# taipingeric/yolo-v4-tf.keras

Measured on AMD Instinct MI355X. Metric: images/sec end-to-end predict() at 608x608 batch 32; conv MFMA %peak, higher is better.
Workload: dtype bf16

## Files before the change

### yolo-v4-tf.keras_amd/csrc/csp_stage.hip

```cpp
#include "conv_chain.h"

#include "phase_trace.h"

namespace y4 {

#ifdef CS_TRACE
__device__ unsigned long long cs_trace_buf[4 * 8 * 16];
#define CS_TR_WG 8
#define CS_TR_T0 3
#endif

#define CS_SEG(K) do { __builtin_amdgcn_sched_barrier(0); __builtin_amdgcn_s_setprio(K); __builtin_amdgcn_sched_barrier(0); } while (0)

constexpr int CS_W3 = 0;
constexpr int CS_W4 = CS_W3 + 8 * 1024;
constexpr int CS_W2 = CS_W4 + 4 * 1024;
constexpr int CS_W5 = CS_W2 + 8 * 1024;
constexpr int CS_W6 = CS_W5 + 36 * 1024;
constexpr int CS_W7 = CS_W6 + 8 * 1024;
constexpr int CS_WBYTES = CS_W7 + 16 * 1024;
constexpr int CS_A3 = 0, CS_A4 = 128, CS_A2 = 192, CS_A5 = 320, CS_A6 = 448, CS_A7 = 576, CS_AFLOATS = 704;
constexpr int CS_AFF = CS_WBYTES;
constexpr int CS_X1 = CS_AFF + 3 * 1024;
constexpr int CS_HROWS = 336;
constexpr int CS_X4 = CS_X1 + CS_HROWS * 128;
constexpr int CS_LDS = CS_X4 + CS_HROWS * 64;
constexpr int CS_BLOB_BYTES = CS_WBYTES + 3 * 1024;
static_assert(CS_LDS <= 160 * 1024, "LDS budget");
constexpr int CS_WAVES = 8, CS_T = 16, CS_H = CS_T + 2;

struct CspStageK {
    const char* in;
    char* out;
    const char* blob;
    int in_cstride, in_coff, out_cstride, out_coff;
    unsigned in_bytes;
    int N, H, W;
    int tiles_x, tiles_y, tiles_per_img, ntiles;
};

template <int NC>
__device__ __forceinline__ void cs_affine(const float* tab, int cout, int fg, float* sc, float* sh) {
#pragma unroll
    for (int c = 0; c < NC; ++c) {
        const int ch = chunk_channel(0, c, fg);
#pragma unroll
        for (int h = 0; h < 8; h += 4) {
            const f32x4 s4 = *(const f32x4*)(tab + ch + h);
            const f32x4 h4 = *(const f32x4*)(tab + cout + ch + h);
#pragma unroll
            for (int e = 0; e < 4; ++e) { sc[c * 8 + h + e] = s4[e]; sh[c * 8 + h + e] = h4[e]; }
        }
    }
}

template <int NREP>
__device__ __forceinline__ void cs_wfrag(const char* w, int s, int lane, u32x4 (&wf)[NREP]) {
#pragma unroll
    for (int j = 0; j < NREP; ++j) wf[j] = *(const u32x4*)(w + ((s * NREP + j) * 64 + lane) * 16);
}

template <int DT, int NREP>
__device__ __forceinline__ void cs_act_pack(const f32x4 (&acc)[NREP], const float* sc, const float* sh, u32x4* out) {
    float v[NREP * 4];
#pragma unroll
    for (int j = 0; j < NREP; ++j)
        bn_act4<true, Y4_ACT_MISH>(acc[j], sc + j * 4, sh + j * 4, v + j * 4);
#pragma unroll
    for (int c = 0; c < NREP / 2; ++c) Elem<DT>::store_chunk(&out[c], v + c * 8);
}

template <int DT>
__global__ __launch_bounds__(64 * CS_WAVES, 1) void csp_stage_kernel(const CspStageK p) {
    using E = Elem<DT>;
    using T = typename E::type;
    extern __shared__ __attribute__((aligned(16))) char smem[];
    const int tid = threadIdx.x, lane = tid & 63, wave = __builtin_amdgcn_readfirstlane(tid >> 6);
    const int q = lane & 15, g = lane >> 4;
    const float* const aff = (const float*)(smem + CS_AFF);
    char* const X1 = smem + CS_X1;
    char* const X4 = smem + CS_X4;

    const int G = gridDim.x, xcd = blockIdx.x & 7, bi = blockIdx.x >> 3;
    const int nb_x = (G - xcd + 7) >> 3;
    const int t_lo = (int)((int64_t)p.ntiles * xcd / 8), t_hi = (int)((int64_t)p.ntiles * (xcd + 1) / 8);
    int t = t_lo + bi;

    {
        const __amdgpu_buffer_rsrc_t rb = make_rsrc(p.blob, CS_BLOB_BYTES);
        for (int u = wave; u < CS_BLOB_BYTES / 1024; u += CS_WAVES)
            buffer_load16_lds(rb, smem + __builtin_amdgcn_readfirstlane(u * 1024), u * 1024 + lane * 16, 0);
    }
    const __amdgpu_buffer_rsrc_t rs_in = make_rsrc(p.in, p.in_bytes);
    constexpr int CS_NPIECE = (CS_HROWS / 8 + CS_WAVES - 1) / CS_WAVES;
    int lx_rel[CS_NPIECE];
#pragma unroll
    for (int k = 0; k < CS_NPIECE; ++k) {
        const int hp = (wave + CS_WAVES * k) * 8 + (lane >> 3);
        const int hy = hp / CS_H, hx = hp - hy * CS_H;
        const int flags = hp >= CS_H * CS_H ? 15 : ((hy == 0) | ((hy == CS_H - 1) << 1) | ((hx == 0) << 2) | ((hx == CS_H - 1) << 3));
        lx_rel[k] = (((hy * p.W + hx) * p.in_cstride + (((lane & 7) ^ (hp & 7)) * 8)) * 2) | flags;
    }
    auto load_x = [&](int tile) {
        const int n = tile / p.tiles_per_img, rem = tile - n * p.tiles_per_img;
        const int ty = rem / p.tiles_x, tx = rem - ty * p.tiles_x;
        const int base = (((n * p.H + ty * CS_T - 1) * p.W + tx * CS_T - 1) * p.in_cstride + p.in_coff) * 2;
        const int tmask = (ty == 0) | ((ty == p.tiles_y - 1) << 1) | ((tx == 0) << 2) | ((tx == p.tiles_x - 1) << 3);
#pragma unroll
        for (int k = 0; k < CS_NPIECE; ++k) {
            const int u = wave + CS_WAVES * k;
            if (u >= CS_HROWS / 8) break;
            const int off = (lx_rel[k] & tmask) || (lx_rel[k] & 15) == 15 ? (int)0x80000000 : base + (lx_rel[k] & ~15);
            buffer_load16_lds(rs_in, X1 + __builtin_amdgcn_readfirstlane(u * 1024), off, 0);
        }
    };
    if (t < t_hi) load_x(t);

    int xr_main[2];
#pragma unroll
    for (int i = 0; i < 2; ++i) xr_main[i] = (2 * wave + i + 1) * CS_H + 1 + q;
    auto ring_geom = [&](int e, int& hy, int& hx) {
        if (e < 2) { hy = e == 0 ? 0 : CS_H - 1; hx = 1 + q; }
        else {
            const int pp = min((e - 2) * 16 + q, 2 * CS_H - 1);
            hy = pp >> 1; hx = (pp & 1) * (CS_H - 1);
        }
    };
    const int n_extra = wave == 0 ? 2 : wave < 4 ? 1 : 0;

    bool first_tile = true;
#ifdef CS_TRACE
    int tr_i = 0;
    unsigned long long tr_t[16] = {0, 0, 0, 0, 0, 0, 0, 0, 0, 0, 0, 0, 0, 0, 0, 0};
#endif
    for (; t < t_hi; t += nb_x) {
        const int n = t / p.tiles_per_img, rem = t - n * p.tiles_per_img;
        const int ty = rem / p.tiles_x, tx = rem - ty * p.tiles_x;
#ifdef CS_TRACE
        const bool tr_on = blockIdx.x == CS_TR_WG && tr_i >= CS_TR_T0 && tr_i < CS_TR_T0 + 4;
#endif
        PHASE_POINT(0);
        if (first_tile) wait_vmcnt_then_barrier<0>();
        else wait_vmcnt_then_barrier<0>();
        first_tile = false;
        PHASE_POINT(1);
        CS_SEG(3);

        u32x4 C2[2][2], R3[2][2];
        {
            float sc3[16], sh3[16], sc4[8], sh4[8];
            cs_affine<2>(aff + CS_A3, 64, g, sc3, sh3);
            cs_affine<1>(aff + CS_A4, 32, g, sc4, sh4);
            f32x4 a3[2][4], a2[2][4];
#pragma unroll
            for (int i = 0; i < 2; ++i)
#pragma unroll
                for (int j = 0; j < 4; ++j) a3[i][j] = a2[i][j] = f32x4{0.f, 0.f, 0.f, 0.f};
#pragma unroll
            for (int s = 0; s < 2; ++s) {
                u32x4 xf[2], w3[4], w2[4];
#pragma unroll
                for (int i = 0; i < 2; ++i) xf[i] = *(const u32x4*)(X1 + xr_main[i] * 128 + (((s * 4 + g) ^ (xr_main[i] & 7)) * 16));
                cs_wfrag<4>(smem + CS_W3, s, lane, w3);
                cs_wfrag<4>(smem + CS_W2, s, lane, w2);
#pragma unroll
                for (int i = 0; i < 2; ++i)
#pragma unroll
                    for (int j = 0; j < 4; ++j) {
                        Mma<DT>::run(a3[i][j], w3[j], xf[i]);
                        Mma<DT>::run(a2[i][j], w2[j], xf[i]);
                    }
            }
            PHASE_POINT(2);
#pragma unroll
            for (int i = 0; i < 2; ++i) cs_act_pack<DT, 4>(a3[i], sc3, sh3, R3[i]);
            {
                float sc2[16], sh2[16];
                cs_affine<2>(aff + CS_A2, 64, g, sc2, sh2);
#pragma unroll
                for (int i = 0; i < 2; ++i) cs_act_pack<DT, 4>(a2[i], sc2, sh2, C2[i]);
            }
            PHASE_POINT(3);
            CS_SEG(2);
            auto conv4_to_t4 = [&](const u32x4* x3, int xr, int hy, int hx) {
                f32x4 a4[2];
                a4[0] = a4[1] = f32x4{0.f, 0.f, 0.f, 0.f};
#pragma unroll
                for (int s = 0; s < 2; ++s) {
                    u32x4 w4[2];
                    cs_wfrag<2>(smem + CS_W4, s, lane, w4);
#pragma unroll
                    for (int j = 0; j < 2; ++j) Mma<DT>::run(a4[j], w4[j], x3[s]);
                }
                u32x4 pk;
                cs_act_pack<DT, 2>(a4, sc4, sh4, &pk);
                const int gy = ty * CS_T - 1 + hy, gx = tx * CS_T - 1 + hx;
                if (!((unsigned)gy < (unsigned)p.H && (unsigned)gx < (unsigned)p.W)) pk = u32x4{0u, 0u, 0u, 0u};
                *(u32x4*)(X4 + xr * 64 + ((g ^ ((xr >> 1) & 3)) * 16)) = pk;
            };
            for (int ex = 0; ex < n_extra; ++ex) {
                int ex_hy, ex_hx;
                ring_geom(ex == 1 ? 4 : wave, ex_hy, ex_hx);
                const int xr_extra = ex_hy * CS_H + ex_hx;
                u32x4 X3e[2];
                f32x4 a3e[4];
#pragma unroll
                for (int j = 0; j < 4; ++j) a3e[j] = f32x4{0.f, 0.f, 0.f, 0.f};
#pragma unroll
                for (int s = 0; s < 2; ++s) {
                    u32x4 w3[4];
                    const u32x4 xf = *(const u32x4*)(X1 + xr_extra * 128 + (((s * 4 + g) ^ (xr_extra & 7)) * 16));
                    cs_wfrag<4>(smem + CS_W3, s, lane, w3);
#pragma unroll
                    for (int j = 0; j < 4; ++j) Mma<DT>::run(a3e[j], w3[j], xf);
                }
                cs_act_pack<DT, 4>(a3e, sc3, sh3, X3e);
                conv4_to_t4(X3e, xr_extra, ex_hy, ex_hx);
            }
            PHASE_POINT(4);
            CS_SEG(1);
#pragma unroll
            for (int i = 0; i < 2; ++i) conv4_to_t4(R3[i], xr_main[i], 2 * wave + i + 1, 1 + q);
        }
        PHASE_POINT(5);
        asm volatile("s_waitcnt lgkmcnt(0)\n\ts_barrier" ::: "memory");
        PHASE_POINT(6);
        CS_SEG(3);
        if (t + nb_x < t_hi) load_x(t + nb_x);
        PHASE_POINT(7);

        {
            f32x4 a5[2][4];
#pragma unroll
            for (int i = 0; i < 2; ++i)
#pragma unroll
                for (int j = 0; j < 4; ++j) a5[i][j] = f32x4{0.f, 0.f, 0.f, 0.f};
#pragma unroll
            for (int tap = 0; tap < 9; ++tap) {
                const int ky = tap / 3, kx = tap - ky * 3;
                u32x4 xf[2], w5[4];
#pragma unroll
                for (int i = 0; i < 2; ++i) {
                    const int r = (2 * wave + i + ky) * CS_H + q + kx;
                    xf[i] = *(const u32x4*)(X4 + r * 64 + ((g ^ ((r >> 1) & 3)) * 16));
                }
                cs_wfrag<4>(smem + CS_W5, tap, lane, w5);
#pragma unroll
                for (int i = 0; i < 2; ++i)
#pragma unroll
                    for (int j = 0; j < 4; ++j) Mma<DT>::run(a5[i][j], w5[j], xf[i]);
            }
            PHASE_POINT(8);
            u32x4 X5[2][2];
            {
                float sc5[16], sh5[16];
                cs_affine<2>(aff + CS_A5, 64, g, sc5, sh5);
#pragma unroll
                for (int i = 0; i < 2; ++i) {
                    float v[16];
#pragma unroll
                    for (int j = 0; j < 4; ++j)
                        bn_act4<true, Y4_ACT_MISH>(a5[i][j], sc5 + j * 4, sh5 + j * 4, v + j * 4);
#pragma unroll
                    for (int c = 0; c < 2; ++c) {
                        float rv[8];
                        E::load_chunk(&R3[i][c], rv);
#pragma unroll
                        for (int e = 0; e < 8; ++e) v[c * 8 + e] += rv[e];
                    }
#pragma unroll
                    for (int c = 0; c < 2; ++c) E::store_chunk(&X5[i][c], v + c * 8);
                }
            }
            PHASE_POINT(9);
            CS_SEG(2);
            u32x4 Y6[2][2];
            {
                f32x4 a6[2][4];
#pragma unroll
                for (int i = 0; i < 2; ++i)
#pragma unroll
                    for (int j = 0; j < 4; ++j) a6[i][j] = f32x4{0.f, 0.f, 0.f, 0.f};
#pragma unroll
                for (int s = 0; s < 2; ++s) {
                    u32x4 w6[4];
                    cs_wfrag<4>(smem + CS_W6, s, lane, w6);
#pragma unroll
                    for (int i = 0; i < 2; ++i)
#pragma unroll
                        for (int j = 0; j < 4; ++j) Mma<DT>::run(a6[i][j], w6[j], X5[i][s]);
                }
                float sc6[16], sh6[16];
                cs_affine<2>(aff + CS_A6, 64, g, sc6, sh6);
#pragma unroll
                for (int i = 0; i < 2; ++i) cs_act_pack<DT, 4>(a6[i], sc6, sh6, Y6[i]);
            }
            PHASE_POINT(10);
            CS_SEG(1);
            {
                f32x4 a7[2][4];
#pragma unroll
                for (int i = 0; i < 2; ++i)
#pragma unroll
                    for (int j = 0; j < 4; ++j) a7[i][j] = f32x4{0.f, 0.f, 0.f, 0.f};
#pragma unroll
                for (int s = 0; s < 4; ++s) {
                    u32x4 w7[4];
                    cs_wfrag<4>(smem + CS_W7, s, lane, w7);
#pragma unroll
                    for (int i = 0; i < 2; ++i)
#pragma unroll
                        for (int j = 0; j < 4; ++j) Mma<DT>::run(a7[i][j], w7[j], s < 2 ? Y6[i][s] : C2[i][s - 2]);
                }
                PHASE_POINT(11);
                float sc7[16], sh7[16];
                cs_affine<2>(aff + CS_A7, 64, g, sc7, sh7);
#pragma unroll
                for (int i = 0; i < 2; ++i) {
                    u32x4 Z[2];
                    cs_act_pack<DT, 4>(a7[i], sc7, sh7, Z);
                    const int64_t pix = ((int64_t)n * p.H + ty * CS_T + 2 * wave + i) * p.W + tx * CS_T + q;
                    T* op = (T*)p.out + pix * p.out_cstride + p.out_coff;
#pragma unroll
                    for (int c = 0; c < 2; ++c) *(u32x4*)(op + chunk_channel(0, c, g)) = Z[c];
                }
            }
        }
        PHASE_POINT(12);
#ifdef CS_TRACE
        if (tr_on && lane == 0) {
#pragma unroll
            for (int k = 0; k < 13; ++k) cs_trace_buf[((tr_i - CS_TR_T0) * 8 + wave) * 16 + k] = tr_t[k];
        }
        ++tr_i;
#endif
    }
}

PHASE_TRACE_READER(y4_cs_trace_read, cs_trace_buf)

bool csp_stage_supported(int dtype, int h, int w) {
    return dtype != Y4_F32 && h % CS_T == 0 && w % CS_T == 0 && h >= CS_T && w >= CS_T;
}
size_t csp_stage_blob_bytes() { return CS_BLOB_BYTES; }

int csp_stage_launch(int dtype, const void* in, int n, int h, int w, int in_cstride, int in_coff, const void* blob, void* out,
                     int out_cstride, int out_coff, hipStream_t stream) {
    Y4_REQUIRE(csp_stage_supported(dtype, h, w), Y4_EINVAL, "csp_stage: dtype %d / %d x %d map not supported", dtype, h, w);
    Y4_REQUIRE(in && blob && out && n > 0, Y4_EINVAL, "csp_stage: null pointer / empty batch");
    Y4_REQUIRE(in_cstride % 8 == 0 && in_coff % 8 == 0 && out_cstride % 8 == 0 && out_coff % 8 == 0, Y4_EINVAL,
               "csp_stage: views not 16-byte aligned");
    const int64_t in_bytes = (int64_t)n * h * w * in_cstride * 2;
    Y4_REQUIRE(in_bytes < (1ll << 31), Y4_EINVAL, "csp_stage: input (%lld B) exceeds the 2 GiB buffer-descriptor range", (long long)in_bytes);
    CspStageK k{};
    k.in = (const char*)in; k.out = (char*)out; k.blob = (const char*)blob;
    k.in_cstride = in_cstride; k.in_coff = in_coff; k.out_cstride = out_cstride; k.out_coff = out_coff;
    k.in_bytes = (unsigned)in_bytes;
    k.N = n; k.H = h; k.W = w;
    k.tiles_x = w / CS_T; k.tiles_y = h / CS_T; k.tiles_per_img = k.tiles_x * k.tiles_y; k.ntiles = n * k.tiles_per_img;
    int cus = 0;
    if (int r = cu_count(&cus)) return r;
    int grid = cus & ~7;
    if (grid < 8) grid = 8;
    if (grid > ((k.ntiles + 7) & ~7)) grid = (k.ntiles + 7) & ~7;
    return dtype == Y4_BF16 ? launch_lds<csp_stage_kernel<Y4_BF16>>(CS_LDS, dim3(grid), dim3(64 * CS_WAVES), CS_LDS, stream, k)
                            : launch_lds<csp_stage_kernel<Y4_F16>>(CS_LDS, dim3(grid), dim3(64 * CS_WAVES), CS_LDS, stream, k);
}

int pack_csp_stage(int dtype, const float* const* w, const float* const* scale, const float* const* shift, void* blob,
                   hipStream_t stream) {
    Y4_REQUIRE(dtype == Y4_BF16 || dtype == Y4_F16, Y4_EINVAL, "pack_csp_stage: 16-bit dtypes only (got %d)", dtype);
    struct Item { int conv, cout, cin, ksize, woff, aoff; };
    static const Item items[6] = {{2, 64, 64, 1, CS_W2, CS_A2},  {3, 64, 64, 1, CS_W3, CS_A3}, {4, 32, 64, 1, CS_W4, CS_A4},
                                  {5, 64, 32, 3, CS_W5, CS_A5},  {6, 64, 64, 1, CS_W6, CS_A6}, {7, 64, 128, 1, CS_W7, CS_A7}};
    for (int k = 0; k < 6; ++k) {
        const Item& it = items[k];
        Y4_REQUIRE(w[k] && scale[k] && shift[k], Y4_EINVAL, "pack_csp_stage: null pointer for conv %d", it.conv);
        if (int r = pack_frag16(dtype, it.cout, it.cin, it.ksize, w[k], (char*)blob + it.woff, stream)) return r;
        if (int r = copy_affine(it.cout, {scale[k], shift[k]}, (float*)((char*)blob + CS_AFF) + it.aoff, stream)) return r;
    }
    return Y4_OK;
}

}
```

### yolo-v4-tf.keras_amd/csrc/phase_trace.h

```cpp
#pragma once

#if defined(RB_TRACE) || defined(CS_TRACE) || defined(SD_TRACE)
#define PHASE_POINT(P)                                                                                      \
    do {                                                                                                    \
        __builtin_amdgcn_sched_barrier(0);                                                                  \
        if (tr_on) asm volatile("s_memtime %0" : "=s"(tr_t[P]));                                            \
        __builtin_amdgcn_sched_barrier(0);                                                                  \
    } while (0)
#define PHASE_TRACE_READER(NAME, BUF) \
    extern "C" int NAME(unsigned long long* dst) { return (int)hipMemcpyFromSymbol(dst, HIP_SYMBOL(BUF), sizeof(BUF)); }
#else
#define PHASE_POINT(P)
#define PHASE_TRACE_READER(NAME, BUF)
#endif
```

### yolo-v4-tf.keras_amd/csrc/resblock.hip

```cpp
#include <type_traits>

#include "conv_chain.h"

#include "phase_trace.h"

namespace y4 {

#ifdef RB_TRACE
__device__ unsigned long long rb_trace_buf[3 * 8 * 16];
#define RB_TR_WG 8
#define RB_TR_T0 1
#endif

constexpr int RB_T = 16, RB_H = RB_T + 2, RB_WAVES = 8;

template <int C, int TY = RB_T> struct RbGeom {
    static constexpr int HR = TY + 2;
    static constexpr int HROWS = HR * RB_H;
    static constexpr int NFA = HR + (2 * HR + 15) / 16;
    static constexpr int CPR = C / 8;
    static constexpr int ROWB = C * 2 + 16;
    static constexpr int XT_PIECES = (HROWS * (CPR + 1) + 63) / 64;
    static constexpr int NF = C / 16;
    static constexpr int KS1 = C / 32;
    static constexpr int STEP_BYTES = 2 * NF * 1024;
    static constexpr int P = KS1 / 2;
    static constexpr int NSTEPS = 10 * P;
    static constexpr int RING = 4;
    static constexpr int PPW = STEP_BYTES / 1024 / RB_WAVES;
    static constexpr int AFF_BYTES = 4 * C * 4;
    static constexpr int AFF_PAD = (AFF_BYTES + 1023) / 1024 * 1024;
    static constexpr int BLOB_BYTES = AFF_PAD + NSTEPS * STEP_BYTES;
    static constexpr int L_AFF = 0, L_RING = AFF_PAD, L_XT = L_RING + RING * STEP_BYTES;
    static constexpr int XT_SLACK = XT_PIECES * 1024 - HROWS * (CPR + 1) * 16;
    static constexpr int LDS = L_XT + XT_PIECES * 1024 + (XT_SLACK >= TOUCH_LDS ? 0 : 1024);
    static constexpr int L_TOUCH = LDS - TOUCH_LDS;
    static constexpr int WN = NF / 4, WM = RB_WAVES / WN, MREP = TY / WM;
    static_assert(C != 64 || 2 * LDS <= 160 * 1024, "C = 64: two workgroups per compute unit (resblock_dispatch)");
    static_assert(LDS <= 160 * 1024 && MREP >= 1 && MREP * WM == TY && PPW >= 1 && PPW * RB_WAVES * 1024 == STEP_BYTES && NFA <= 3 * RB_WAVES,
                  "resblock geometry");
};

struct ResBlockK {
    const char* in;
    char* out;
    const char* blob;
    int in_cstride, in_coff, out_cstride, out_coff;
    unsigned in_bytes, out_bytes;
    int N, H, W;
    int tiles_x, tiles_y, tiles_per_img, ntiles;
    int t_begin, t_end;
    int touch;
};

template <int DT, int C, int TY>
__global__ __launch_bounds__(64 * RB_WAVES, C == 64 ? 4 : 2) void resblock_kernel(const ResBlockK p) {
    using E = Elem<DT>;
    using G = RbGeom<C, TY>;
    constexpr int PARTS = RB_T / TY;
    constexpr int ROWB = G::ROWB, CPR = G::CPR, NF = G::NF, MREP = G::MREP;
    extern __shared__ __attribute__((aligned(16))) char smem[];
    const int tid = threadIdx.x, lane = tid & 63, wave = __builtin_amdgcn_readfirstlane(tid >> 6);
    const int q = lane & 15, g = lane >> 4;
    const int wm = wave / G::WN, wn = wave - wm * G::WN;
    const float* const aff = (const float*)(smem + G::L_AFF);
    char* const XT = smem + G::L_XT;
    char* const ring = smem + G::L_RING;

    const int GR = gridDim.x, xcd = blockIdx.x & 7, bi = blockIdx.x >> 3;
    const int nb_x = (GR - xcd + 7) >> 3;
    const int span = p.t_end - p.t_begin;
    const int t_lo = p.t_begin + (int)((int64_t)span * xcd / 8), t_hi = p.t_begin + (int)((int64_t)span * (xcd + 1) / 8);
    int t = t_lo + bi;
    auto locate = [&](int u, int& n, int& y_out0, int& tx) {
        const int full = u / PARTS, part = u - full * PARTS;
        n = full / p.tiles_per_img;
        const int rem = full - n * p.tiles_per_img, ty = rem / p.tiles_x;
        tx = rem - ty * p.tiles_x;
        y_out0 = ty * RB_T + part * TY;
    };

    const __amdgpu_buffer_rsrc_t rb = make_rsrc(p.blob, G::BLOB_BYTES);
    const __amdgpu_buffer_rsrc_t rs_in = make_rsrc(p.in, p.in_bytes), rs_out = make_rsrc(p.out, p.out_bytes);
    if (p.touch != 0) weight_touch(rb, smem + G::L_TOUCH, 0, G::BLOB_BYTES, wave, RB_WAVES, lane);
    for (int u = wave; u < G::AFF_PAD / 1024; u += RB_WAVES)
        buffer_load16_lds(rb, smem + __builtin_amdgcn_readfirstlane(u * 1024), u * 1024 + lane * 16, 0);
    auto stage_w = [&](int st) {
        char* const dst = ring + (st & (G::RING - 1)) * G::STEP_BYTES;
#pragma unroll
        for (int k = 0; k < G::PPW; ++k) {
            const int u = wave + k * RB_WAVES;
            buffer_load16_lds(rb, dst + __builtin_amdgcn_readfirstlane(u * 1024), G::AFF_PAD + u * 1024 + lane * 16, st * G::STEP_BYTES);
        }
    };
    auto load_x = [&](int tile) {
        int n, yo, tx;
        locate(tile, n, yo, tx);
        const int y0 = yo - 1, x0 = tx * RB_T - 1;
        constexpr int SPR = CPR + 1, DSLOT = RB_WAVES * 64, DHP = DSLOT / SPR, DCH = DSLOT % SPR, DHY = DHP / RB_H, DHX = DHP % RB_H;
        static_assert(DCH + SPR - 1 < 2 * SPR && DHX + RB_H < 2 * RB_H, "one carry per step");
        int slot0 = wave * 64 + lane;
        asm volatile("" : "+v"(slot0));
        const int hp0 = slot0 / SPR;
        int ch = slot0 - hp0 * SPR, hy = hp0 / RB_H;
        int hx = hp0 - hy * RB_H;
        const int pix_b = p.in_cstride * 2, row_b = p.W * pix_b;
        int off = (((n * p.H + y0) * p.W + x0) * p.in_cstride + p.in_coff) * 2 + hy * row_b + hx * pix_b + ch * 16;
        const int d_off = DHY * row_b + DHX * pix_b + DCH * 16, c_ch = pix_b - SPR * 16, c_hx = row_b - RB_H * pix_b;
#pragma unroll
        for (int k = 0; k * RB_WAVES < G::XT_PIECES; ++k) {
            const int u = wave + k * RB_WAVES;
            if (u < G::XT_PIECES) {
                const bool ok = ch < CPR && hy < G::HR && (unsigned)(y0 + hy) < (unsigned)p.H && (unsigned)(x0 + hx) < (unsigned)p.W;
                buffer_load16_lds(rs_in, XT + __builtin_amdgcn_readfirstlane(u * 1024), ok ? off : (int)0x80000000, 0);
            }
            ch += DCH; hx += DHX; hy += DHY; off += d_off;
            if (ch >= SPR) { ch -= SPR; hx += 1; off += c_ch; }
            if (hx >= RB_H) { hx -= RB_H; hy += 1; off += c_hx; }
        }
    };
    if (t < t_hi) { load_x(t); stage_w(0); stage_w(1); stage_w(2); stage_w(3); }

#ifdef RB_TRACE
    int tr_i = 0;
    unsigned long long tr_t[16] = {0, 0, 0, 0, 0, 0, 0, 0, 0, 0, 0, 0, 0, 0, 0, 0};
#endif
    for (; t < t_hi; t += nb_x) {
        int n, y_out0, tx;
        locate(t, n, y_out0, tx);
#ifdef RB_TRACE
        const bool tr_on = TY == RB_T && C == RB_TRACE && blockIdx.x == RB_TR_WG && tr_i >= RB_TR_T0 && tr_i < RB_TR_T0 + 3;
#endif
        PHASE_POINT(0);
        wait_vmcnt_then_barrier<0>();
        PHASE_POINT(1);

        u32x4 res[MREP][2];

        auto phase_a = [&](auto nfr_c) {
            constexpr int NFR = decltype(nfr_c)::value;
            char* row[NFR];
            bool inside[NFR];
#pragma unroll
            for (int k = 0; k < NFR; ++k) {
                const int f = wave + k * RB_WAVES;
                int hy, hx;
                if (f < G::HR) { hy = f; hx = 1 + q; }
                else { const int pp = min((f - G::HR) * 16 + q, 2 * G::HR - 1); hy = pp >> 1; hx = (pp & 1) * (RB_H - 1); }
                const int r = hy * RB_H + hx;
                row[k] = XT + r * ROWB;
                const int gy = y_out0 - 1 + hy, gx = tx * RB_T - 1 + hx;
                inside[k] = (unsigned)gy < (unsigned)p.H && (unsigned)gx < (unsigned)p.W;
            }
            f32x4 acc[NFR][NF];
#pragma unroll
            for (int k = 0; k < NFR; ++k)
#pragma unroll
                for (int j = 0; j < NF; ++j) acc[k][j] = f32x4{0.f, 0.f, 0.f, 0.f};
#pragma unroll
            for (int s = 0; s < G::KS1; ++s) {
                u32x4 xf[NFR], wf[NF];
#pragma unroll
                for (int k = 0; k < NFR; ++k) xf[k] = *(const u32x4*)(row[k] + (s * 4 + g) * 16);
#pragma unroll
                for (int j = 0; j < NF; ++j) wf[j] = *(const u32x4*)(ring + (s >> 1) * G::STEP_BYTES + (((s & 1) * NF + j) * 64 + lane) * 16);
#pragma unroll
                for (int k = 0; k < NFR; ++k)
#pragma unroll
                    for (int j = 0; j < NF; ++j) Mma<DT>::run(acc[k][j], wf[j], xf[k]);
            }
#pragma unroll
            for (int c = 0; c < NF / 2; ++c) {
                float sc[8], sh[8];
#pragma unroll
                for (int h = 0; h < 8; h += 4) {
                    const int ch = chunk_channel(0, c, g) + h;
                    const f32x4 s4 = *(const f32x4*)(aff + ch), h4 = *(const f32x4*)(aff + C + ch);
#pragma unroll
                    for (int e = 0; e < 4; ++e) { sc[h + e] = s4[e]; sh[h + e] = h4[e]; }
                }
#pragma unroll
                for (int k = 0; k < NFR; ++k) {
                    float v[8];
                    bn_act4<true, Y4_ACT_MISH>(acc[k][2 * c], sc, sh, v);
                    bn_act4<true, Y4_ACT_MISH>(acc[k][2 * c + 1], sc + 4, sh + 4, v + 4);
                    u32x4 pk;
                    E::store_chunk(&pk, v);
                    if (!inside[k]) pk = u32x4{0u, 0u, 0u, 0u};
                    *(u32x4*)(row[k] + (4 * c + g) * 16) = pk;
                }
            }
        };
        if (wave + 2 * RB_WAVES < G::NFA) phase_a(std::integral_constant<int, 3>{});
        else if (wave + RB_WAVES < G::NFA) phase_a(std::integral_constant<int, 2>{});
        else if (wave < G::NFA) phase_a(std::integral_constant<int, 1>{});
        PHASE_POINT(2);
        asm volatile("s_waitcnt lgkmcnt(0)\n\ts_barrier" ::: "memory");
        PHASE_POINT(3);

        {
            int pix[MREP];
#pragma unroll
            for (int i = 0; i < MREP; ++i) {
                const int gy = y_out0 + wm * MREP + i, gx = tx * RB_T + q;
                pix[i] = gy < p.H && gx < p.W ? (n * p.H + gy) * p.W + gx : -1;
            }
            auto load_res = [&]() {
#pragma unroll
                for (int i = 0; i < MREP; ++i) {
                    const int o = pix[i] < 0 ? (int)0x80000000 : (pix[i] * p.in_cstride + p.in_coff) * 2;
#pragma unroll
                    for (int c = 0; c < 2; ++c) res[i][c] = buffer_load16(rs_in, o + chunk_channel(wn * 64, c, g) * 2);
                }
            };
            constexpr int S0 = G::NSTEPS - 4, RES_LOADS = 2 * MREP;
            f32x4 acc[MREP][4];
#pragma unroll
            for (int i = 0; i < MREP; ++i)
#pragma unroll
                for (int j = 0; j < 4; ++j) acc[i][j] = f32x4{0.f, 0.f, 0.f, 0.f};
#pragma unroll
            for (int st = 4; st <= G::P + 3; ++st) stage_w(st);
            const char* const xbase = XT + ((wm * MREP) * RB_H + q) * ROWB + g * 16;
            u32x4 xf[2][MREP], wf[2][4];
            auto read_frags = [&](int buf, int st, int kk) {
                const int ks = st - G::P;
                const int cb = ks / 9, tap = ks - cb * 9;
                const int ky = tap / 3, kx = tap - ky * 3;
                const char* const wst = ring + (st & (G::RING - 1)) * G::STEP_BYTES;
#pragma unroll
                for (int i = 0; i < MREP; ++i) {
                    xf[buf][i] = *(const u32x4*)(xbase + ((i + ky) * RB_H + kx) * ROWB + (cb * 8 + kk * 4) * 16);
                }
#pragma unroll
                for (int j = 0; j < 4; ++j) wf[buf][j] = *(const u32x4*)(wst + ((kk * NF + wn * 4 + j) * 64 + lane) * 16);
            };
            auto mma = [&](int buf) {
#pragma unroll
                for (int i = 0; i < MREP; ++i)
#pragma unroll
                    for (int j = 0; j < 4; ++j)
                        Mma<DT>::run(acc[i][j], wf[buf][j], xf[buf][i]);
            };
            PHASE_POINT(4);
            read_frags(0, G::P, 0);
#pragma unroll
            for (int st = G::P; st < G::NSTEPS; ++st) {
                if (st == G::P + 3 * G::P) PHASE_POINT(5);
                if (st == G::P + 6 * G::P) PHASE_POINT(6);
                if (st == S0) load_res();
                read_frags(1, st, 1);
                __builtin_amdgcn_sched_barrier(0);
                mma(0);
                __builtin_amdgcn_sched_barrier(0);
                if (st + 1 < G::NSTEPS) {
                    constexpr int LAST = G::NSTEPS - 1;
                    const int younger = (st + 3 < LAST ? st + 3 : LAST) - (st + 1);
                    const int extra = st >= S0 && st <= S0 + 2 ? RES_LOADS : 0;
                    static_assert(S0 > G::P && 2 * G::PPW + RES_LOADS < 64, "window of the residual's loads");
                    wait_vmcnt_lgkm_then_barrier_n<2 * G::PPW + RES_LOADS>(younger == 0 ? 0 : (younger >= 2 ? 2 : 1) * G::PPW + extra);
                    if (st + 4 < G::NSTEPS) stage_w(st + 4);
                    read_frags(0, st + 1, 0);
                    __builtin_amdgcn_sched_barrier(0);
                }
                mma(1);
                __builtin_amdgcn_sched_barrier(0);
            }
            PHASE_POINT(7);
            asm volatile("s_waitcnt lgkmcnt(0)\n\ts_barrier" ::: "memory");
            PHASE_POINT(8);
#pragma unroll
            for (int i = 0; i < MREP; ++i)
#pragma unroll
                for (int c = 0; c < 2; ++c) asm volatile("" : "+v"(res[i][c]));
            const bool more = t + nb_x < t_hi;
            if (more) { load_x(t + nb_x); stage_w(0); stage_w(1); stage_w(2); stage_w(3); }
            PHASE_POINT(9);
            float sc3[16], sh3[16];
#pragma unroll
            for (int c = 0; c < 2; ++c)
#pragma unroll
                for (int h = 0; h < 8; h += 4) {
                    const int ch = chunk_channel(wn * 64, c, g) + h;
                    const f32x4 s4 = *(const f32x4*)(aff + 2 * C + ch), h4 = *(const f32x4*)(aff + 3 * C + ch);
#pragma unroll
                    for (int e = 0; e < 4; ++e) { sc3[c * 8 + h + e] = s4[e]; sh3[c * 8 + h + e] = h4[e]; }
                }
#pragma unroll
            for (int i = 0; i < MREP; ++i) {
                float v[16];
#pragma unroll
                for (int j = 0; j < 4; ++j) bn_act4<true, Y4_ACT_MISH>(acc[i][j], sc3 + j * 4, sh3 + j * 4, v + j * 4);
                const int o = pix[i] < 0 ? (int)0x80000000 : (pix[i] * p.out_cstride + p.out_coff) * 2;
#pragma unroll
                for (int c = 0; c < 2; ++c) {
                    float rv[8];
                    E::load_chunk(&res[i][c], rv);
#pragma unroll
                    for (int e = 0; e < 8; ++e) v[c * 8 + e] += rv[e];
                    u32x4 pk;
                    E::store_chunk(&pk, v + c * 8);
                    buffer_store16<0>(rs_out, pk, o + chunk_channel(wn * 64, c, g) * 2);
                }
            }
        }
        PHASE_POINT(10);
#ifdef RB_TRACE
        if (tr_on && lane == 0) {
#pragma unroll
            for (int k = 0; k < 11; ++k) rb_trace_buf[((tr_i - RB_TR_T0) * 8 + wave) * 16 + k] = tr_t[k];
        }
        ++tr_i;
#endif
    }
}

PHASE_TRACE_READER(y4_rb_trace_read, rb_trace_buf)

bool resblock_supported(int dtype, int c) { return dtype != Y4_F32 && (c == 128 || c == 64); }
size_t resblock_blob_bytes(int c) { return c == 128 ? RbGeom<128>::BLOB_BYTES : RbGeom<64>::BLOB_BYTES; }

template <int DT, int C, int TY>
static int resblock_run(const ResBlockK& k, int slots, hipStream_t stream) {
    int grid = slots;
    const int span = k.t_end - k.t_begin;
    if (grid > ((span + 7) & ~7)) grid = (span + 7) & ~7;
    if (grid < 8) grid = 8;
    constexpr int lds = RbGeom<C, TY>::LDS;
    return launch_lds<resblock_kernel<DT, C, TY>>(lds, dim3(grid), dim3(64 * RB_WAVES), lds, stream, k);
}

static bool rb_parts_enabled() {
    static const bool on = [] { const char* e = getenv("Y4_RB_PARTS"); return !(e && e[0] == '0'); }();
    return on;
}

template <int DT, int C>
static int resblock_dispatch(ResBlockK& k, hipStream_t stream) {
    int cus = 0;
    if (int r = cu_count(&cus)) return r;
    const int slots = (cus & ~7) * (C == 64 ? 2 : 1);
    constexpr int MAXP = C == 128 ? 4 : 2;
    const int full = k.ntiles / slots * slots, rem = k.ntiles - full;
    int parts = 1;
    if (rb_parts_enabled() && rem > 0)
        for (int pp = 2; pp <= MAXP; pp *= 2)
            if (rem * pp <= slots) parts = pp;
    if (parts == 1) {
        k.t_begin = 0; k.t_end = k.ntiles;
        return resblock_run<DT, C, RB_T>(k, slots, stream);
    }
    if (full > 0) {
        k.t_begin = 0; k.t_end = full;
        if (int r = resblock_run<DT, C, RB_T>(k, slots, stream)) return r;
    }
    k.t_begin = full * parts; k.t_end = k.ntiles * parts;
    if (parts == 2) return resblock_run<DT, C, RB_T / 2>(k, slots, stream);
    if constexpr (MAXP >= 4) return resblock_run<DT, C, RB_T / 4>(k, slots, stream);
    return Y4_EINVAL;
}

int resblock_launch(int dtype, int c, const void* in, int n, int h, int w, int in_cstride, int in_coff, const void* blob, void* out,
                    int out_cstride, int out_coff, hipStream_t stream) {
    Y4_REQUIRE(resblock_supported(dtype, c), Y4_EINVAL, "resblock: dtype %d / %d channels not supported", dtype, c);
    Y4_REQUIRE(in && blob && out && n > 0 && h > 0 && w > 0, Y4_EINVAL, "resblock: null pointer / empty batch");
    Y4_REQUIRE(in_cstride % 8 == 0 && in_coff % 8 == 0 && out_cstride % 8 == 0 && out_coff % 8 == 0, Y4_EINVAL,
               "resblock: views not 16-byte aligned");
    const int64_t in_bytes = (int64_t)n * h * w * in_cstride * 2;
    const int64_t out_bytes = (int64_t)n * h * w * out_cstride * 2;
    Y4_REQUIRE(in_bytes < (1ll << 31) && out_bytes < (1ll << 31), Y4_EINVAL,
               "resblock: input (%lld B) or output (%lld B) exceeds the 2 GiB buffer-descriptor range", (long long)in_bytes, (long long)out_bytes);
    ResBlockK k{};
    k.in = (const char*)in; k.out = (char*)out; k.blob = (const char*)blob;
    k.in_cstride = in_cstride; k.in_coff = in_coff; k.out_cstride = out_cstride; k.out_coff = out_coff;
    k.in_bytes = (unsigned)in_bytes; k.out_bytes = (unsigned)out_bytes;
    k.N = n; k.H = h; k.W = w;
    k.touch = weight_touch_enabled() ? 1 : 0;
    k.tiles_x = (w + RB_T - 1) / RB_T; k.tiles_y = (h + RB_T - 1) / RB_T; k.tiles_per_img = k.tiles_x * k.tiles_y; k.ntiles = n * k.tiles_per_img;
    if (c == 128) return dtype == Y4_BF16 ? resblock_dispatch<Y4_BF16, 128>(k, stream) : resblock_dispatch<Y4_F16, 128>(k, stream);
    return dtype == Y4_BF16 ? resblock_dispatch<Y4_BF16, 64>(k, stream) : resblock_dispatch<Y4_F16, 64>(k, stream);
}

int pack_resblock(int dtype, int c, const float* w1, const float* scale1, const float* shift1, const float* w3, const float* scale3,
                  const float* shift3, void* blob, hipStream_t stream) {
    Y4_REQUIRE(resblock_supported(dtype, c) && w1 && w3 && scale1 && shift1 && scale3 && shift3 && blob, Y4_EINVAL, "pack_resblock: bad argument");
    const int w1_bytes = c * c * 2, aff_pad = (4 * c * 4 + 1023) / 1024 * 1024;
    char* b = (char*)blob;
    if (int r = pack_frag16(dtype, c, c, 1, w1, b + aff_pad, stream)) return r;
    if (int r = pack_frag16(dtype, c, c, 3, w3, b + aff_pad + w1_bytes, stream)) return r;
    return copy_affine(c, {scale1, shift1, scale3, shift3}, (float*)b, stream);
}

}
```

Before: 6679.

## Fuse resblock remainder part-tiles into the main launch as leading work

For C=128 resblocks whose tile count leaves a remainder, the remainder split into smaller part-tiles is now processed at the start of the same kernel launch instead of in a second launch. Each workgroup first runs one part-tile (half- or quarter-height) and then moves on to its full tiles, and the full tile's first loads are issued inside the part-tile's pipeline. This removes a launch boundary and the tail idle time between the two launches, at the cost of a more complex templated kernel, and it assumes the part-tile LDS fits inside the full-tile allocation. It also adds trace-only per-workgroup realtime stamps and adds waits to the existing trace points, which compile out by default.

```diff
diff --git a/yolo-v4-tf.keras_amd/csrc/csp_stage.hip b/yolo-v4-tf.keras_amd/csrc/csp_stage.hip
--- a/yolo-v4-tf.keras_amd/csrc/csp_stage.hip
+++ b/yolo-v4-tf.keras_amd/csrc/csp_stage.hip
@@ -6,6 +6,7 @@
 
 #ifdef CS_TRACE
 __device__ unsigned long long cs_trace_buf[4 * 8 * 16];
+__device__ unsigned long long cs_wg_buf[PHASE_WG_N * PHASE_WG_TILES * PHASE_WG_POINTS];
 #define CS_TR_WG 8
 #define CS_TR_T0 3
 #endif
@@ -132,11 +133,14 @@
 #ifdef CS_TRACE
     int tr_i = 0;
     unsigned long long tr_t[16] = {0, 0, 0, 0, 0, 0, 0, 0, 0, 0, 0, 0, 0, 0, 0, 0};
+    unsigned long long wg_t[PHASE_WG_POINTS] = {0, 0, 0, 0};
 #endif
     for (; t < t_hi; t += nb_x) {
         const int n = t / p.tiles_per_img, rem = t - n * p.tiles_per_img;
         const int ty = rem / p.tiles_x, tx = rem - ty * p.tiles_x;
 #ifdef CS_TRACE
+        const bool wg_on = wave == 0 && blockIdx.x % PHASE_WG_STRIDE == 0 && blockIdx.x / PHASE_WG_STRIDE < PHASE_WG_N &&
+                           tr_i >= CS_TR_T0 && tr_i < CS_TR_T0 + PHASE_WG_TILES;
         const bool tr_on = blockIdx.x == CS_TR_WG && tr_i >= CS_TR_T0 && tr_i < CS_TR_T0 + 4;
 #endif
         PHASE_POINT(0);
@@ -144,6 +148,7 @@
         else wait_vmcnt_then_barrier<0>();
         first_tile = false;
         PHASE_POINT(1);
+        PHASE_WG_STAMP(0);
         CS_SEG(3);
 
         u32x4 C2[2][2], R3[2][2];
@@ -225,9 +230,11 @@
         PHASE_POINT(5);
         asm volatile("s_waitcnt lgkmcnt(0)\n\ts_barrier" ::: "memory");
         PHASE_POINT(6);
+        PHASE_WG_STAMP(1);
         CS_SEG(3);
         if (t + nb_x < t_hi) load_x(t + nb_x);
         PHASE_POINT(7);
+        PHASE_WG_STAMP(2);
 
         {
             f32x4 a5[2][4];
@@ -327,7 +334,13 @@
             }
         }
         PHASE_POINT(12);
+        PHASE_WG_STAMP(3);
 #ifdef CS_TRACE
+        if (wg_on && lane == 0) {
+#pragma unroll
+            for (int k = 0; k < PHASE_WG_POINTS; ++k)
+                cs_wg_buf[(blockIdx.x / PHASE_WG_STRIDE * PHASE_WG_TILES + tr_i - CS_TR_T0) * PHASE_WG_POINTS + k] = wg_t[k];
+        }
         if (tr_on && lane == 0) {
 #pragma unroll
             for (int k = 0; k < 13; ++k) cs_trace_buf[((tr_i - CS_TR_T0) * 8 + wave) * 16 + k] = tr_t[k];
@@ -338,6 +351,9 @@
 }
 
 PHASE_TRACE_READER(y4_cs_trace_read, cs_trace_buf)
+#ifdef CS_TRACE
+PHASE_TRACE_READER(y4_cs_wg_read, cs_wg_buf)
+#endif
 
 bool csp_stage_supported(int dtype, int h, int w) {
     return dtype != Y4_F32 && h % CS_T == 0 && w % CS_T == 0 && h >= CS_T && w >= CS_T;
diff --git a/yolo-v4-tf.keras_amd/csrc/phase_trace.h b/yolo-v4-tf.keras_amd/csrc/phase_trace.h
--- a/yolo-v4-tf.keras_amd/csrc/phase_trace.h
+++ b/yolo-v4-tf.keras_amd/csrc/phase_trace.h
@@ -4,12 +4,20 @@
 #define PHASE_POINT(P)                                                                                      \
     do {                                                                                                    \
         __builtin_amdgcn_sched_barrier(0);                                                                  \
-        if (tr_on) asm volatile("s_memtime %0" : "=s"(tr_t[P]));                                            \
+        if (tr_on) asm volatile("s_memtime %0\n\ts_waitcnt lgkmcnt(0)" : "=s"(tr_t[P]));                       \
         __builtin_amdgcn_sched_barrier(0);                                                                  \
     } while (0)
 #define PHASE_TRACE_READER(NAME, BUF) \
     extern "C" int NAME(unsigned long long* dst) { return (int)hipMemcpyFromSymbol(dst, HIP_SYMBOL(BUF), sizeof(BUF)); }
+constexpr int PHASE_WG_STRIDE = 17, PHASE_WG_N = 16, PHASE_WG_TILES = 8, PHASE_WG_POINTS = 4;
+#define PHASE_WG_STAMP(K)                                                                                   \
+    do {                                                                                                    \
+        __builtin_amdgcn_sched_barrier(0);                                                                  \
+        if (wg_on) asm volatile("s_memrealtime %0\n\ts_waitcnt lgkmcnt(0)" : "=s"(wg_t[K]));                 \
+        __builtin_amdgcn_sched_barrier(0);                                                                  \
+    } while (0)
 #else
 #define PHASE_POINT(P)
+#define PHASE_WG_STAMP(K)
 #define PHASE_TRACE_READER(NAME, BUF)
 #endif
diff --git a/yolo-v4-tf.keras_amd/csrc/resblock.hip b/yolo-v4-tf.keras_amd/csrc/resblock.hip
--- a/yolo-v4-tf.keras_amd/csrc/resblock.hip
+++ b/yolo-v4-tf.keras_amd/csrc/resblock.hip
@@ -8,6 +8,7 @@
 
 #ifdef RB_TRACE
 __device__ unsigned long long rb_trace_buf[3 * 8 * 16];
+__device__ unsigned long long rb_wg_buf[PHASE_WG_N * PHASE_WG_TILES * PHASE_WG_POINTS];
 #define RB_TR_WG 8
 #define RB_TR_T0 1
 #endif
@@ -50,15 +51,16 @@
     int N, H, W;
     int tiles_x, tiles_y, tiles_per_img, ntiles;
     int t_begin, t_end;
+    int p_begin, p_end;
     int touch;
 };
 
-template <int DT, int C, int TY>
+template <int DT, int C, int TY, int TYP = 0>
 __global__ __launch_bounds__(64 * RB_WAVES, C == 64 ? 4 : 2) void resblock_kernel(const ResBlockK p) {
     using E = Elem<DT>;
     using G = RbGeom<C, TY>;
-    constexpr int PARTS = RB_T / TY;
-    constexpr int ROWB = G::ROWB, CPR = G::CPR, NF = G::NF, MREP = G::MREP;
+    static_assert(TYP == 0 || (TYP < TY && RbGeom<C, TYP == 0 ? TY : TYP>::LDS <= G::LDS), "the leading part tile fits the LDS of the tiles behind it");
+    constexpr int ROWB = G::ROWB, CPR = G::CPR, NF = G::NF;
     extern __shared__ __attribute__((aligned(16))) char smem[];
     const int tid = threadIdx.x, lane = tid & 63, wave = __builtin_amdgcn_readfirstlane(tid >> 6);
     const int q = lane & 15, g = lane >> 4;
@@ -72,12 +74,13 @@
     const int span = p.t_end - p.t_begin;
     const int t_lo = p.t_begin + (int)((int64_t)span * xcd / 8), t_hi = p.t_begin + (int)((int64_t)span * (xcd + 1) / 8);
     int t = t_lo + bi;
-    auto locate = [&](int u, int& n, int& y_out0, int& tx) {
+    auto locate = [&](auto rows_c, int u, int& n, int& y_out0, int& tx) {
+        constexpr int ROWS = decltype(rows_c)::value, PARTS = RB_T / ROWS;
         const int full = u / PARTS, part = u - full * PARTS;
         n = full / p.tiles_per_img;
         const int rem = full - n * p.tiles_per_img, ty = rem / p.tiles_x;
         tx = rem - ty * p.tiles_x;
-        y_out0 = ty * RB_T + part * TY;
+        y_out0 = ty * RB_T + part * ROWS;
     };
 
     const __amdgpu_buffer_rsrc_t rb = make_rsrc(p.blob, G::BLOB_BYTES);
@@ -93,9 +96,10 @@
             buffer_load16_lds(rb, dst + __builtin_amdgcn_readfirstlane(u * 1024), G::AFF_PAD + u * 1024 + lane * 16, st * G::STEP_BYTES);
         }
     };
-    auto load_x = [&](int tile) {
+    auto load_x = [&](auto rows_c, int tile) {
+        using GT = RbGeom<C, decltype(rows_c)::value>;
         int n, yo, tx;
-        locate(tile, n, yo, tx);
+        locate(rows_c, tile, n, yo, tx);
         const int y0 = yo - 1, x0 = tx * RB_T - 1;
         constexpr int SPR = CPR + 1, DSLOT = RB_WAVES * 64, DHP = DSLOT / SPR, DCH = DSLOT % SPR, DHY = DHP / RB_H, DHX = DHP % RB_H;
         static_assert(DCH + SPR - 1 < 2 * SPR && DHX + RB_H < 2 * RB_H, "one carry per step");
@@ -108,10 +112,10 @@
         int off = (((n * p.H + y0) * p.W + x0) * p.in_cstride + p.in_coff) * 2 + hy * row_b + hx * pix_b + ch * 16;
         const int d_off = DHY * row_b + DHX * pix_b + DCH * 16, c_ch = pix_b - SPR * 16, c_hx = row_b - RB_H * pix_b;
 #pragma unroll
-        for (int k = 0; k * RB_WAVES < G::XT_PIECES; ++k) {
+        for (int k = 0; k * RB_WAVES < GT::XT_PIECES; ++k) {
             const int u = wave + k * RB_WAVES;
-            if (u < G::XT_PIECES) {
-                const bool ok = ch < CPR && hy < G::HR && (unsigned)(y0 + hy) < (unsigned)p.H && (unsigned)(x0 + hx) < (unsigned)p.W;
+            if (u < GT::XT_PIECES) {
+                const bool ok = ch < CPR && hy < GT::HR && (unsigned)(y0 + hy) < (unsigned)p.H && (unsigned)(x0 + hx) < (unsigned)p.W;
                 buffer_load16_lds(rs_in, XT + __builtin_amdgcn_readfirstlane(u * 1024), ok ? off : (int)0x80000000, 0);
             }
             ch += DCH; hx += DHX; hy += DHY; off += d_off;
@@ -119,21 +123,30 @@
             if (hx >= RB_H) { hx -= RB_H; hy += 1; off += c_hx; }
         }
     };
-    if (t < t_hi) { load_x(t); stage_w(0); stage_w(1); stage_w(2); stage_w(3); }
+    const std::integral_constant<int, TY> ty_c{};
+    auto first_loads = [&]() { if (t < t_hi) { load_x(ty_c, t); stage_w(0); stage_w(1); stage_w(2); stage_w(3); } };
 
 #ifdef RB_TRACE
     int tr_i = 0;
     unsigned long long tr_t[16] = {0, 0, 0, 0, 0, 0, 0, 0, 0, 0, 0, 0, 0, 0, 0, 0};
+    int wg_i = 0;
+    unsigned long long wg_t[PHASE_WG_POINTS] = {0, 0, 0, 0};
 #endif
-    for (; t < t_hi; t += nb_x) {
+    auto run_tile = [&](auto rows_c, int t, auto issue_next) __attribute__((always_inline)) {
+        constexpr int ROWS = decltype(rows_c)::value;
+        using G = RbGeom<C, ROWS>;
+        constexpr int MREP = G::MREP;
         int n, y_out0, tx;
-        locate(t, n, y_out0, tx);
+        locate(rows_c, t, n, y_out0, tx);
 #ifdef RB_TRACE
-        const bool tr_on = TY == RB_T && C == RB_TRACE && blockIdx.x == RB_TR_WG && tr_i >= RB_TR_T0 && tr_i < RB_TR_T0 + 3;
+        const bool wg_on = TY == RB_T && C == RB_TRACE && wave == 0 && blockIdx.x % PHASE_WG_STRIDE == 0 &&
+                           blockIdx.x / PHASE_WG_STRIDE < PHASE_WG_N && wg_i < PHASE_WG_TILES;
+        const bool tr_on = ROWS == RB_T && TY == RB_T && C == RB_TRACE && blockIdx.x == RB_TR_WG && tr_i >= RB_TR_T0 && tr_i < RB_TR_T0 + 3;
 #endif
         PHASE_POINT(0);
         wait_vmcnt_then_barrier<0>();
         PHASE_POINT(1);
+        PHASE_WG_STAMP(0);
 
         u32x4 res[MREP][2];
 
@@ -269,13 +282,14 @@
             PHASE_POINT(7);
             asm volatile("s_waitcnt lgkmcnt(0)\n\ts_barrier" ::: "memory");
             PHASE_POINT(8);
+            PHASE_WG_STAMP(1);
 #pragma unroll
             for (int i = 0; i < MREP; ++i)
 #pragma unroll
                 for (int c = 0; c < 2; ++c) asm volatile("" : "+v"(res[i][c]));
-            const bool more = t + nb_x < t_hi;
-            if (more) { load_x(t + nb_x); stage_w(0); stage_w(1); stage_w(2); stage_w(3); }
+            issue_next();
             PHASE_POINT(9);
+            PHASE_WG_STAMP(2);
             float sc3[16], sh3[16];
 #pragma unroll
             for (int c = 0; c < 2; ++c)
@@ -305,29 +319,52 @@
             }
         }
         PHASE_POINT(10);
+        PHASE_WG_STAMP(3);
 #ifdef RB_TRACE
+        if (wg_on && lane == 0) {
+#pragma unroll
+            for (int k = 0; k < PHASE_WG_POINTS; ++k)
+                rb_wg_buf[(blockIdx.x / PHASE_WG_STRIDE * PHASE_WG_TILES + wg_i) * PHASE_WG_POINTS + k] = wg_t[k];
+        }
+        ++wg_i;
         if (tr_on && lane == 0) {
 #pragma unroll
             for (int k = 0; k < 11; ++k) rb_trace_buf[((tr_i - RB_TR_T0) * 8 + wave) * 16 + k] = tr_t[k];
         }
-        ++tr_i;
+        if (ROWS == TY) ++tr_i;
 #endif
-    }
+    };
+
+    if constexpr (TYP != 0) {
+        const std::integral_constant<int, TYP> typ_c{};
+        const int pspan = p.p_end - p.p_begin;
+        const int u_lo = p.p_begin + (int)((int64_t)pspan * xcd / 8), u_hi = p.p_begin + (int)((int64_t)pspan * (xcd + 1) / 8);
+        const int u = u_lo + ((bi & 1) ? ((nb_x + 1) >> 1) + (bi >> 1) : bi >> 1);
+        if (u < u_hi) {
+            load_x(typ_c, u); stage_w(0); stage_w(1); stage_w(2); stage_w(3);
+            run_tile(typ_c, u, first_loads);
+        } else first_loads();
+    } else first_loads();
+    for (; t < t_hi; t += nb_x)
+        run_tile(ty_c, t, [&]() { if (t + nb_x < t_hi) { load_x(ty_c, t + nb_x); stage_w(0); stage_w(1); stage_w(2); stage_w(3); } });
 }
 
 PHASE_TRACE_READER(y4_rb_trace_read, rb_trace_buf)
+#ifdef RB_TRACE
+PHASE_TRACE_READER(y4_rb_wg_read, rb_wg_buf)
+#endif
 
 bool resblock_supported(int dtype, int c) { return dtype != Y4_F32 && (c == 128 || c == 64); }
 size_t resblock_blob_bytes(int c) { return c == 128 ? RbGeom<128>::BLOB_BYTES : RbGeom<64>::BLOB_BYTES; }
 
-template <int DT, int C, int TY>
+template <int DT, int C, int TY, int TYP = 0>
 static int resblock_run(const ResBlockK& k, int slots, hipStream_t stream) {
     int grid = slots;
     const int span = k.t_end - k.t_begin;
     if (grid > ((span + 7) & ~7)) grid = (span + 7) & ~7;
     if (grid < 8) grid = 8;
     constexpr int lds = RbGeom<C, TY>::LDS;
-    return launch_lds<resblock_kernel<DT, C, TY>>(lds, dim3(grid), dim3(64 * RB_WAVES), lds, stream, k);
+    return launch_lds<resblock_kernel<DT, C, TY, TYP>>(lds, dim3(grid), dim3(64 * RB_WAVES), lds, stream, k);
 }
 
 static bool rb_parts_enabled() {
@@ -349,6 +386,13 @@
     if (parts == 1) {
         k.t_begin = 0; k.t_end = k.ntiles;
         return resblock_run<DT, C, RB_T>(k, slots, stream);
+    }
+    if (full > 0 && C == 128) {
+        k.t_begin = 0; k.t_end = full;
+        k.p_begin = full * parts; k.p_end = k.ntiles * parts;
+        if (parts == 2) return resblock_run<DT, C, RB_T, RB_T / 2>(k, slots, stream);
+        if constexpr (MAXP >= 4) return resblock_run<DT, C, RB_T, RB_T / 4>(k, slots, stream);
+        return Y4_EINVAL;
     }
     if (full > 0) {
         k.t_begin = 0; k.t_end = full;
```

Measured after the change: 6669. No clear change (-0.2%).
